# Lab-LVM/imagenet-models

Hardware: AMD Instinct MI355X
Metric: images/sec (whole node) GA-ConvNeXt-T 3x224x224 bf16 training step (higher is better)
Workload: dtype bf16; 1 GPU; ga_convnext_tiny_768 train step (fwd + GA loss lam=-0.8 + bwd + all-reduce + adamw lr=0), batch 256/GPU, drop_path 0.2, synthetic 3x224x224; global_batch=256, parallelism=dp1, dist_backend=none, grad_exchange=torch, allreduce_buckets=0

## Files before the change

imagenet-models_amd/_lib.py:

```python
import ctypes as C
import os

_HERE = os.path.dirname(os.path.abspath(__file__))
LIB_PATH = os.environ.get('GAEXT_LIB') or os.path.join(_HERE, 'csrc', 'libgaext.so')

GA_F32, GA_BF16 = 0, 1
ACT_NONE, ACT_GELU, ACT_RELU = 0, 1, 2
A_PLAIN, A_PATCH2, A_STEM4_NCHW, A_CONV3, A_CONV3S2, A_NEIGH2 = 0, 1, 2, 3, 4, 5
C_PLAIN, C_UNPATCH2 = 0, 1

vp, i32, i64, f32 = C.c_void_p, C.c_int, C.c_int64, C.c_float


class GemmDesc(C.Structure):
    _fields_ = [
        ('M', i32), ('N', i32), ('K', i32), ('batch', i32), ('dtype', i32),
        ('A', vp), ('lda', i64), ('strideA', i64), ('a_batch_mod', i32), ('a_kind', i32),
        ('a_H', i32), ('a_W', i32), ('a_C', i32), ('a_act', i32),
        ('B', vp), ('ldb', i64), ('strideB', i64),
        ('C', vp), ('ldc', i64), ('strideC', i64), ('c_kind', i32),
        ('c_H', i32), ('c_W', i32), ('c_C', i32), ('c_f32', i32), ('C2', vp), ('c2_mode', i32),
        ('alpha', f32), ('bias', vp), ('strideBias', i64), ('act', i32),
        ('H', vp), ('ldh', i64), ('strideH', i64), ('h_is_deriv', i32),
        ('rowscale', vp), ('rows_per_scale', i32),
# ... 123 lines not shown
    'ga_layernorm_bwd_dp': ([vp, vp, vp, vp, vp, vp, vp, vp, vp, i64, i32, i32, vp, vp, i64, i32, vp], i32),
    'ga_bn_finalize': ([vp, vp, i64, vp, vp, f32, f32, vp, vp, vp, vp, vp, vp, i32, i32, vp], i32),
    'ga_affine_act': ([vp, vp, vp, vp, vp, i64, vp, i64, i32, i32, i32, i64, vp], i32),
    'ga_bn_bwd_reduce': ([vp, vp, vp, vp, vp, vp, i64, vp, vp, i64, i32, i32, i64, vp], i32),
    'ga_bn_bwd_apply': ([vp, vp, vp, vp, vp, vp, vp, vp, vp, i64, i64, vp, i64, i32, i32, i64, i64, vp], i32),
    'ga_pool_concat_fwd': ([vp, vp, i32, i32, i32, i32, i32, i32, i32, i32, i32, i32, vp], i32),
    'ga_pool_concat_bwd': ([vp, vp, vp, i32, i32, i32, i32, i32, i32, i32, i32, i32, i32, vp], i32),
    'ga_spatial_sum': ([vp, vp, vp, i32, i32, i32, f32, i32, vp], i32),
    'ga_se_mlp_fwd': ([vp, vp, vp, vp, vp, vp, vp, i32, i32, i32, vp], i32),
    'ga_se_mlp_bwd': ([vp, vp, vp, vp, vp, vp, vp, f32, vp, vp, vp, vp, i32, i32, i32, vp], i32),
    'ga_chan_scale': ([vp, vp, vp, vp, i32, i32, i32, i32, vp], i32),
    'ga_gram_pack_fwd': ([vp, vp, vp, i32, i32, i32, i32, i32, vp], i32),
    'ga_gram_pack_bwd': ([vp, vp, vp, vp, i32, i32, i32, i32, i32, vp], i32),
    'ga_gram_f64_fwd_workspace': ([i32, i32], C.c_size_t),
    'ga_gram_f64_bwd_workspace': ([i32, i32], C.c_size_t),
    'ga_gram_f64_fwd': ([vp, vp, vp, vp, C.c_size_t, i32, i32, i32, i32, i32, i32, i32, vp], i32),
    'ga_gram_f64_bwd': ([vp, vp, vp, vp, vp, vp, C.c_size_t, i32, i32, i32, i32, i32, i32, i32, vp], i32),
    'ga_token_cat': ([vp, vp, vp, i32, i32, i32, i32, vp], i32),
    'ga_token_split': ([vp, vp, vp, i32, i32, i32, i32, i32, i32, vp], i32),
    'ga_class_attn_fwd': ([vp, vp, vp, vp, i32, i32, i32, i32, f32, i32, vp], i32),
    'ga_class_attn_bwd': ([vp, vp, vp, vp, vp, vp, i32, i32, i32, i32, f32, i32, vp], i32),
    'ga_class_attn_fwd2': ([vp, vp, vp, i64, vp, vp, i32, i32, i32, i32, f32, i32, vp], i32),
    'ga_class_attn_bwd2': ([vp, vp, vp, vp, i64, vp, vp, vp, vp, i32, i32, i32, i32, f32, i32, vp], i32),
    'ga_loss_fwd_bwd': ([vp, vp, vp, vp, i32, i32, i32, f32, i32, f32, f32, i32, vp], i32),
    'ga_heads_topk': ([vp, i32, i32, i32, i32, vp, vp, vp], i32),
    'ga_sgd_step': ([vp, vp, vp, vp, i64, i32, f32, vp], i32),
    'ga_adamw_step': ([vp, vp, vp, vp, vp, i64, f32, vp], i32),
    'ga_weight_prep_batch': ([vp, i32, vp], i32),
    'ga_weight_unfold_batch': ([vp, i32, vp], i32),
    'ga_small_batch': ([vp, i32, vp], i32),
    'ga_cswin_attn_fwd': ([C.POINTER(CswinAttnDesc), vp], i32),
    'ga_cswin_attn_bwd_workspace': ([C.POINTER(CswinAttnDesc)], C.c_size_t),
    'ga_cswin_attn_bwd': ([C.POINTER(CswinAttnDesc), vp, vp, vp, C.c_size_t, vp], i32),
    'ga_cswin_lepe_wgrad_reduce': ([C.POINTER(CswinAttnDesc), vp, vp, vp, vp, vp, vp], i32),
    'ga_cswin_lepe_wgrad': ([C.POINTER(CswinAttnDesc), vp, vp, vp, vp, vp, vp], i32),
    'ga_layernorm_gelu_fwd': ([vp, vp, vp, vp, vp, vp, i64, i32, f32, i32, vp], i32),
    'ga_layernorm_gelu_bwd': ([vp, vp, vp, vp, vp, vp, vp, vp, vp, i64, i32, i32, vp], i32),
    'ga_nchw3_to_nhwc8': ([vp, vp, i32, i32, i32, i32, vp], i32),
    'ga_convw_pack': ([vp, vp, i32, i32, i32, i32, i64, i32, vp], i32),
    'ga_convw_unpack_grad': ([vp, vp, i32, i32, i32, i32, i64, vp], i32),
    'ga_conv3s2_dgrad_prep': ([vp, vp, i32, i32, i64, i32, vp], i32),
    'ga_gram_pack_fwd2': ([vp, vp, vp, i32, i32, i32, i32, i32, i32, vp], i32),
    'ga_gram_pack_bwd2': ([vp, vp, vp, vp, i32, i32, i32, i32, i32, i32, vp], i32),
    'ga_map_tokens_fwd': ([vp, vp, i32, i32, i32, i32, i32, vp], i32),
    'ga_map_tokens_bwd': ([vp, vp, i32, i32, i32, i32, i32, vp], i32),
    'ga_class_attn_mt_fwd': ([vp, vp, vp, i64, vp, vp, vp, i32, i32, i32, i32, i32, f32, i32, vp], i32),
    'ga_class_attn_mt_bwd': ([vp, vp, vp, vp, i64, vp, vp, vp, vp, vp, i64, i32, i32, i32, i32, i32, f32, i32, vp], i32),
    'ga_class_attn_mt_ia_fwd': ([vp, vp, vp, i64, vp, vp, vp, vp, vp, vp, vp, i32, i32, i32, i32, i32, f32, i32, vp], i32),
    'ga_class_attn_mt_ia_bwd': ([vp, vp, vp, vp, i64, vp, vp, vp, vp, vp, vp, vp, vp, i64, vp, vp, vp, vp, i32, i32, i32, i32, i32, f32, i32,
                                 vp], i32),
    'ga_map_loss_fwd_bwd': ([vp, vp, vp, vp, vp, vp, i32, i32, i32, f32, i32, f32, f32, i32, vp], i32),
    'ga_gelu_fwd': ([vp, vp, i64, i32, vp], i32),
    'ga_gelu_bwd': ([vp, vp, vp, i64, i32, vp], i32),
    'ga_relu_drop': ([vp, vp, vp, vp, i64, i32, vp], i32),
    'ga_mask_mul': ([vp, vp, vp, vp, i64, i32, vp], i32),
    'ga_copy2d': ([vp, i64, vp, i64, i64, i32, i32, i32, vp], i32),
    'ga_dropout_mask_sample': ([vp, i64, f32, C.c_uint64, vp, vp], i32),
    'ga_drop_path_sample': ([vp, vp, i32, i32, C.c_uint64, vp, vp], i32),
    'ga_loss_dense_fwd_bwd': ([vp, vp, vp, vp, vp, vp, vp, i32, i32, i32, f32, i32, f32, f32, f32, i32, vp], i32),
    'ga_u8_normalize': ([vp, vp, i32, i32, i32, i32, C.POINTER(f32), C.POINTER(f32), vp], i32),
    'ga_input_erase': ([vp, i32, vp, i32, i32, i32, i32, C.POINTER(f32), C.POINTER(f32), vp, i32, i32, C.c_uint64, C.c_uint64, vp], i32),
    'ga_input_collate': ([vp, i32, vp, i32, i32, i32, i32, C.POINTER(f32), C.POINTER(f32), vp, vp, i32, i32, C.c_uint64, C.c_uint64, vp],
                         i32),
    'ga_mixup_target_elem': ([vp, vp, i32, i32, vp, C.c_double, vp], i32),
    'ga_rand_augment': ([vp, vp, vp, C.c_size_t, i32, i32, i32, i32, vp, i32, vp, vp], i32),
    'ga_rand_augment_work_bytes': ([i32, i32, i32, i32, i32], C.c_size_t),
    'ga_rand_augment_check_table': ([vp, i32], i32),
    'ga_resize_crop': ([vp, C.c_uint64, vp, vp, vp, C.c_size_t, i32, i32, i32, vp], i32),
    'ga_resize_crop_work_bytes': ([vp, i32, i32, i32], C.c_size_t),
    'ga_resize_crop_check_table': ([vp, i32, i32, i32, C.c_uint64], i32),
    'ga_resample_coeffs': ([i32, i32, i32, vp, vp, i32, vp], i32),
    'ga_jpeg_probe': ([vp, C.c_size_t, vp], i32),
    'ga_jpeg_entropy_decode': ([vp, C.c_size_t, vp, C.c_size_t, vp], i32),
    'ga_jpeg_check_table': ([vp, i32, C.c_uint64, C.c_uint64, C.c_uint64, C.c_uint64], i32),
    'ga_jpeg_work_bytes': ([vp, i32], C.c_size_t),
    'ga_jpeg_reconstruct': ([vp, i32, vp, vp, vp, vp, vp], i32),
    'ga_mixup_batch': ([vp, vp, i32, i32, i32, i32, C.c_double, i32, i32, i32, i32, i32, vp], i32),
    'ga_mixup_target': ([vp, vp, i32, i32, C.c_double, C.c_double, vp], i32),
    'ga_agc_clip': ([vp, vp, vp, i32, f32, f32, vp], i32),
    'ga_small_linear_fwd': ([C.POINTER(SmallLinearDesc), vp], i32),
    'ga_small_linear_bwd': ([C.POINTER(SmallLinearDesc), vp, vp, i32, vp, vp, vp, vp], i32),
    'ga_colstats': ([vp, i64, i32, i32, vp, vp, i32, vp], i32),
    'ga_pad_copy_f32': ([vp, vp, i64, i64, i64, i64, i32, vp], i32),
    'ga_pad_copy': ([vp, vp, i64, i64, i64, i64, i32, i32, vp], i32),
    'ga_stem4_ln_fwd': ([vp, vp, i64, vp, vp, vp, vp, vp, vp, vp, i32, i32, i32, i32, f32, vp], i32),
    'ga_blockdiag_f32': ([vp, vp, i64, i32, i32, i32, i64, i32, i32, vp], i32),
    'ga_pad_groups_f32': ([vp, vp, i64, i64, i32, i32, i32, i32, i32, i32, vp], i32),
    'ga_attn_fwd': ([C.POINTER(AttnDesc), vp], i32),
    'ga_attn_bwd_workspace': ([C.POINTER(AttnDesc)], C.c_size_t),
    'ga_attn_bwd': ([C.POINTER(AttnDesc), vp, vp, vp, C.c_size_t, vp], i32),
    'ga_patchify': ([vp, vp, i32, i32, i32, i32, i32, i32, vp], i32),
    'ga_vit_embed_fwd': ([vp, vp, vp, vp, i32, i32, i32, i32, vp], i32),
    'ga_vit_embed_bwd': ([vp, vp, vp, vp, i32, i32, i32, i32, vp], i32),
    'ga_patchify_strided': ([vp, vp, i32, i32, i32, i32, i32, i32, i32, vp], i32),
    'ga_pos_add_fwd': ([vp, vp, vp, i32, i32, i32, i32, vp], i32),
    'ga_pos_add_bwd': ([vp, vp, i32, i32, i32, i32, vp], i32),
    'ga_dwpool_fwd': ([vp, vp, vp, vp, i32, i32, i32, i32, i32, i32, vp], i32),
    'ga_dwpool_bwd_data': ([vp, vp, vp, i32, i32, i32, i32, i32, i32, vp], i32),
    'ga_dwpool_bwd_weight': ([vp, vp, vp, vp, i32, i32, i32, i32, i32, i32, vp], i32),
    'ga_resize_concat_fwd': ([vp, vp, i32, i32, i32, i32, i32, i32, i64, i32, i32, vp], i32),
    'ga_resize_concat_bwd': ([vp, vp, i32, i32, i32, i32, i32, i32, i64, i32, i32, vp], i32),
    'ga_rows_bcast': ([vp, vp, i32, i32, i32, f32, i32, vp], i32),
    'ga_token_gap_fwd': ([vp, vp, i32, i32, i32, i32, vp], i32),
    'ga_token_gap_bwd': ([vp, vp, i32, i32, i32, i32, vp], i32),
    'ga_mlp_supported': ([i32, i32, i32], i32),
    'ga_mlp_fwd': ([C.POINTER(MlpDesc), vp], i32),
    'ga_mlp_bwd': ([C.POINTER(MlpBwdDesc), vp], i32),
    'ga_mlp_bwd_wgrad_supported': ([i32, i32, i32], i32),
    'ga_mlp_bwd_partials': ([C.POINTER(MlpBwdDesc)], C.c_size_t),
    'ga_memset': ([vp, i32, C.c_size_t, vp], i32),
    'ga_transpose_f32': ([vp, vp, i32, i32, i32, vp], i32),
    'ga_axpy_f32': ([vp, vp, f32, i64, vp], i32),
    'ga_lerp_f32': ([vp, vp, f32, i64, vp], i32),
    'ga_sumsq_f32': ([vp, i64, vp, vp], i32),
    'ga_lamb_stage1': ([vp, vp, vp, vp, vp, vp, vp, vp, i32, vp, vp], i32),
    'ga_lamb_stage2': ([vp, vp, vp, vp, i32, vp, vp], i32),
    'ga_clip_grad_f32': ([vp, i64, vp, f32, i32, vp], i32),
    'ga_rowscale': ([vp, vp, vp, i64, i64, i32, vp], i32),
    'ga_cast_from_f32': ([vp, vp, i64, i32, vp], i32),
    'ga_cast_to_f32': ([vp, vp, i64, i32, vp], i32),
}

_lib = None


def load():
    global _lib
    if _lib is not None:
        return _lib
    if not os.path.exists(LIB_PATH):
        raise RuntimeError(f'libgaext.so not found at {LIB_PATH}: build it with `make -C {os.path.dirname(LIB_PATH)}` '
                           f'(there is no CPU fallback for the product path)')
    lib = C.CDLL(LIB_PATH)
    for name, (argtypes, restype) in _SIGS.items():
        fn = getattr(lib, name)
        fn.argtypes = argtypes
        fn.restype = restype
    _lib = lib
    return lib


def last_error():
    buf = C.create_string_buffer(512)
    load().ga_last_error(buf, 512)
    return buf.value.decode(errors='replace')


def config_string():
    buf = C.create_string_buffer(1024)
    load().ga_config_string(buf, 1024)
    s = buf.value.decode(errors='replace')
    host = sorted(k for k in os.environ if k.startswith(('GAEXT_', 'GA_FUSED_MLP')) and k != 'GAEXT_LIB')
    known = {'GAEXT_ASYNC_WGRAD', 'GAEXT_FWD_SPLIT', 'GAEXT_PAR_BRANCH', 'GAEXT_FWD_SKEW', 'GAEXT_FUSE_DP', 'GAEXT_HEAD_STREAMS',
             'GA_FUSED_MLP', 'GAEXT_SMALL_SINGLE', 'GAEXT_SYNC_DEBUG', 'GAEXT_MLP_WG1', 'GAEXT_MLP_PREFETCH'}
    for k in host:
        if k in known:
            s += f' host:{k}={os.environ[k]}'
    if os.environ.get('GAEXT_LIB'):
        s += f' lib={os.environ["GAEXT_LIB"]}'
    return s


class knobs:

    def __init__(self, **kv):
        self.kv = kv

    def __enter__(self):
        lib = load()
        for k, v in self.kv.items():
            check(lib.ga_set_knob(k.encode(), int(v)), f'ga_set_knob({k})')
        return self

    def __exit__(self, *exc):
        lib = load()
        for k in self.kv:
            lib.ga_unset_knob(k.encode())
        return False


def check(rc, what):
    if rc != 0:
        raise RuntimeError(f'libgaext {what} failed (code {rc}): {last_error()}')


def exported_symbols():
    return sorted(_SIGS)
```

imagenet-models_amd/csrc/wprep.hip:

```cpp
#include <algorithm>
#include "common.h"

namespace {

__device__ __forceinline__ long w_index(int n, int kcol, int Ci, int KH, int KW, int stem, int* ci_out) {
    const int KK = Ci * KH * KW;
    if (stem || (KH == 1 && KW == 1)) {
        *ci_out = stem ? kcol / (KH * KW) : kcol;
        return (long)n * KK + kcol;
    }
    const int tap = kcol / Ci, ci = kcol - tap * Ci;
    *ci_out = ci;
    return ((long)n * Ci + ci) * (KH * KW) + tap;
}

template <typename T>
__global__ __launch_bounds__(256) void wprep_out_kernel(const float* __restrict__ w, const float* __restrict__ rs,
                                                        const float* __restrict__ cs, const int* __restrict__ perm,
                                                        T* __restrict__ out, long ldo, int rows, int Ci, int KH, int KW,
                                                        int stem) {
    const int KK = Ci * KH * KW;
    const long total = (long)rows * ldo;
    for (long i = (long)blockIdx.x * 256 + threadIdx.x; i < total; i += (long)gridDim.x * 256) {
        const int no = (int)(i / ldo), kcol = (int)(i - (long)no * ldo);
// ... 301 lines not shown
            const long t = i / tcols;
            const int r = (int)(t % trows), g = (int)(t / trows);
            float v = 0.f;
            if (!d.flip) {
                if (col < d.Co) {
                    const int n = d.row_perm ? d.row_perm[g * d.Co + col] : g * d.Co + col;
                    int ci;
                    v = d.w[w_index(n, r, d.Ci, d.KH, d.KW, d.stem, &ci)];
                    if (d.rs) v *= d.rs[n];
                    if (d.cs) v *= d.cs[ci];
                }
            } else if (col < d.KH * d.KW * d.Co) {
                const int tapf = col / d.Co, co = col - tapf * d.Co;
                const int tap = d.KH * d.KW - 1 - tapf;
                const int n = d.row_perm ? d.row_perm[g * d.Co + co] : g * d.Co + co;
                v = d.w[((long)n * d.Ci + r) * (d.KH * d.KW) + tap];
                if (d.rs) v *= d.rs[n];
                if (d.cs) v *= d.cs[r];
            }
            elt<T>::st(outT + t * d.ldt + col, v);
        }
    }
}

__global__ __launch_bounds__(256) void wprep_batch_kernel(const ga_wprep_desc* __restrict__ jobs) {
    __shared__ float tile[64][65];
    const ga_wprep_desc d = jobs[blockIdx.y];
    if (wprep_is_1x1(d)) {
        if (d.dtype == GA_BF16) wprep_job_1x1<bf16_t>(d, gridDim.x, blockIdx.x, tile);
        else wprep_job_1x1<float>(d, gridDim.x, blockIdx.x, tile);
        return;
    }
    if (d.dtype == GA_BF16) wprep_job<bf16_t>(d, gridDim.x, blockIdx.x);
    else wprep_job<float>(d, gridDim.x, blockIdx.x);
}

__global__ __launch_bounds__(256) void small_batch_kernel(const ga_small_desc* __restrict__ jobs) {
    const ga_small_desc d = jobs[blockIdx.y];
    if (d.kind == 0) {
        for (long i = (long)blockIdx.x * 256 + threadIdx.x; i < d.n; i += (long)gridDim.x * 256) d.y[i] += d.a * d.x[i];
    } else if (d.kind == 1) {
        const long total = (long)d.R * d.C;
        for (long i = (long)blockIdx.x * 256 + threadIdx.x; i < total; i += (long)gridDim.x * 256) {
            const int c = (int)(i / d.R), r = (int)(i - (long)c * d.R);
            const float v = d.x[(long)r * d.C + c];
            d.y[i] = d.accumulate ? d.y[i] + v : v;
        }
    } else {
        const int lane = threadIdx.x & 63;
        for (int no = blockIdx.x * 4 + (threadIdx.x >> 6); no < d.R; no += gridDim.x * 4) {
            const int n = d.row_perm ? d.row_perm[no] : no;
            float s = 0.f;
            if (d.v) {
                if (d.C % 4 == 0 && ((reinterpret_cast<uintptr_t>(d.x) | reinterpret_cast<uintptr_t>(d.v)) & 15) == 0) {
                    for (int c = lane * 4; c < d.C; c += 256) {
                        float w[4], vv[4];
                        load4(d.x + (long)n * d.C + c, w);
                        load4(d.v + c, vv);
                        s += w[0] * vv[0] + w[1] * vv[1] + w[2] * vv[2] + w[3] * vv[3];
                    }
                } else {
                    for (int c = lane; c < d.C; c += 64) s += d.x[(long)n * d.C + c] * d.v[c];
                }
            }
            s = wave_sum(s);
            if (lane == 0) d.y[no] = (d.rs ? d.rs[n] : 1.f) * ((d.b ? d.b[n] : 0.f) + s);
        }
    }
}

__global__ __launch_bounds__(256) void unfold_batch_kernel(const ga_wunfold_desc* __restrict__ jobs) {
    const ga_wunfold_desc d = jobs[blockIdx.y];
    const int KK = d.Ci * d.KH * d.KW;
    const bool vec4 = d.KH == 1 && d.KW == 1 && !d.stem && KK % 4 == 0 && d.ldg % 4 == 0 &&
                      ((reinterpret_cast<uintptr_t>(d.G) | reinterpret_cast<uintptr_t>(d.dW) |
                        reinterpret_cast<uintptr_t>(d.cs) | reinterpret_cast<uintptr_t>(d.v)) & 15) == 0;
    if (d.dW && vec4) {
        const unsigned P = (unsigned)KK >> 2, total = (unsigned)d.N * P;
        for (unsigned i = blockIdx.x * 256u + threadIdx.x; i < total; i += gridDim.x * 256u) {
            const unsigned no = i / P, k4 = (i - no * P) << 2;
            const int n = d.row_perm ? d.row_perm[no] : (int)no;
            float g[4], w[4];
            load4(d.G + (long)no * d.ldg + k4, g);
            if (d.cs) {
                float cs[4];
                load4(d.cs + k4, cs);
#pragma unroll
                for (int j = 0; j < 4; ++j) g[j] *= cs[j];
            }
            if (d.gb && d.v) {
                float vv[4];
                load4(d.v + k4, vv);
                const float gbn = d.gb[no];
#pragma unroll
                for (int j = 0; j < 4; ++j) g[j] = fmaf(gbn, vv[j], g[j]);
            }
            const float rs = d.rs ? d.rs[n] : 1.f;
            float* dst = d.dW + (long)n * KK + k4;
            load4(dst, w);
#pragma unroll
            for (int j = 0; j < 4; ++j) w[j] = fmaf(g[j], rs, w[j]);
            store4(dst, w);
        }
    } else if (d.dW) {
        const long total = (long)d.N * KK;
        for (long i = (long)blockIdx.x * 256 + threadIdx.x; i < total; i += (long)gridDim.x * 256) {
            const int no = (int)(i / KK), kcol = (int)(i - (long)no * KK);
            const int n = d.row_perm ? d.row_perm[no] : no;
            int ci;
            const long wi = w_index(n, kcol, d.Ci, d.KH, d.KW, d.stem, &ci);
            float val = d.G[(long)no * d.ldg + kcol];
            if (d.cs) val *= d.cs[ci];
            if (d.gb && d.v) val += d.gb[no] * d.v[ci];
            if (d.rs) val *= d.rs[n];
            d.dW[wi] += val;
        }
    }
    if (d.d_rs || (d.db && d.gb)) {
        const int lane = threadIdx.x & 63;
        for (int no = blockIdx.x * 4 + (threadIdx.x >> 6); no < d.N; no += gridDim.x * 4) {
            const int n = d.row_perm ? d.row_perm[no] : no;
            if (d.d_rs) {
                float s = 0.f;
                for (int k = lane; k < KK; k += 64) {
                    int ci;
                    const long wi = w_index(n, k, d.Ci, d.KH, d.KW, d.stem, &ci);
                    s += d.G[(long)no * d.ldg + k] * d.W[wi] * (d.cs ? d.cs[ci] : 1.f);
                    if (d.gb && d.v) s += d.gb[no] * d.W[wi] * d.v[ci];
                }
                s = wave_sum(s);
                if (lane == 0) d.d_rs[n] += s + ((d.gb && d.b) ? d.gb[no] * d.b[n] : 0.f);
            }
            if (d.db && d.gb && lane == 0) d.db[n] += (d.rs ? d.rs[n] : 1.f) * d.gb[no];
        }
    }
    if (d.d_cs || d.d_v) {
        const int rows_per_blk = (d.N + gridDim.x - 1) / gridDim.x;
        const int r0 = blockIdx.x * rows_per_blk, r1 = min(d.N, r0 + rows_per_blk);
        for (int c = threadIdx.x; c < d.Ci; c += 256) {
            float a = 0.f, bs = 0.f;
            for (int n = r0; n < r1; ++n) {
                const float wv = d.W[(long)n * d.Ci + c] * (d.rs ? d.rs[n] : 1.f);
                a += d.G[(long)n * d.ldg + c] * wv;
                if (d.gb) bs += d.gb[n] * wv;
            }
            if (r1 > r0) {
                if (d.d_cs) atomicAdd(d.d_cs + c, a);
                if (d.d_v) atomicAdd(d.d_v + c, bs);
            }
        }
    }
}

int nblocks(long n, int cap = 4096) { return (int)std::max<long>(1, std::min<long>(cap, (n + 255) / 256)); }

}

extern "C" int ga_weight_prep(const ga_wprep_desc* d, ga_stream_t stream) {
    GA_REQUIRE(d && d->w && d->G >= 1 && d->Co >= 1 && d->Ci >= 1 && d->KH >= 1 && d->KW >= 1, "ga_weight_prep: bad args");
    GA_REQUIRE(!(d->cs && d->G > 1), "ga_weight_prep: column scale with groups unsupported");
    GA_REQUIRE(!(d->flip && d->stem), "ga_weight_prep: flip+stem unsupported");
    GA_REQUIRE(d->t_cols == 0 || d->t_cols == d->ldt, "ga_weight_prep: t_cols != ldt needs ga_weight_prep_batch");
    const int KK = d->Ci * d->KH * d->KW;
    hipStream_t s = reinterpret_cast<hipStream_t>(stream);
    if (d->out) {
        GA_REQUIRE(d->ldo >= KK, "ga_weight_prep: ldo < K");
        const long total = (long)d->G * d->Co * d->ldo;
        if (d->dtype == GA_BF16)
            hipLaunchKernelGGL(wprep_out_kernel<bf16_t>, dim3(nblocks(total)), dim3(256), 0, s, d->w, d->rs, d->cs,
                               d->row_perm, (bf16_t*)d->out, (long)d->ldo, d->G * d->Co, d->Ci, d->KH, d->KW, d->stem);
        else
            hipLaunchKernelGGL(wprep_out_kernel<float>, dim3(nblocks(total)), dim3(256), 0, s, d->w, d->rs, d->cs,
                               d->row_perm, (float*)d->out, (long)d->ldo, d->G * d->Co, d->Ci, d->KH, d->KW, d->stem);
    }
    if (d->outT) {
        GA_REQUIRE(d->ldt >= (d->flip ? d->KH * d->KW * d->Co : d->Co), "ga_weight_prep: ldt too small");
        const long total = (long)d->G * (d->flip ? d->Ci : KK) * d->ldt;
        if (d->dtype == GA_BF16)
            hipLaunchKernelGGL(wprep_outT_kernel<bf16_t>, dim3(nblocks(total)), dim3(256), 0, s, d->w, d->rs, d->cs,
                               d->row_perm, (bf16_t*)d->outT, (long)d->ldt, d->G, d->Co, d->Ci, d->KH, d->KW, d->stem, d->flip);
        else
            hipLaunchKernelGGL(wprep_outT_kernel<float>, dim3(nblocks(total)), dim3(256), 0, s, d->w, d->rs, d->cs,
                               d->row_perm, (float*)d->outT, (long)d->ldt, d->G, d->Co, d->Ci, d->KH, d->KW, d->stem, d->flip);
    }
    return ga_check_launch("ga_weight_prep");
}

extern "C" int ga_bias_fold(const float* W, const float* b, const float* rs, const float* v, const int* row_perm,
                            float* be, int N, int C, ga_stream_t stream) {
    GA_REQUIRE(be && N > 0 && (!v || W), "ga_bias_fold: bad args");
    hipLaunchKernelGGL(bias_fold_kernel, dim3(cdiv(N, 4)), dim3(256), 0, reinterpret_cast<hipStream_t>(stream), W, b, rs,
                       v, row_perm, be, N, C);
    return ga_check_launch("ga_bias_fold");
}

extern "C" int ga_weight_unfold(const ga_wunfold_desc* d, ga_stream_t stream) {
    GA_REQUIRE(d && d->G && d->N > 0 && d->Ci > 0, "ga_weight_unfold: bad args");
    GA_REQUIRE(!((d->d_cs || d->d_v || d->v) && (d->KH != 1 || d->KW != 1)),
               "ga_weight_unfold: column grads / bias-fold vector need a 1x1 kernel");
    GA_REQUIRE(!((d->d_rs || d->d_cs || d->d_v) && !d->W), "ga_weight_unfold: W required");
    GA_REQUIRE(!(d->row_perm && (d->d_cs || d->d_v)), "ga_weight_unfold: row_perm with column grads unsupported");
    hipStream_t s = reinterpret_cast<hipStream_t>(stream);
    const int KK = d->Ci * d->KH * d->KW;
    if (d->dW)
        hipLaunchKernelGGL(unfold_dw_kernel, dim3(nblocks((long)d->N * KK)), dim3(256), 0, s, d->G, (long)d->ldg, d->rs,
                           d->cs, d->gb, d->v, d->row_perm, d->dW, d->N, d->Ci, d->KH, d->KW, d->stem);
    if (d->d_rs || (d->db && d->gb))
        hipLaunchKernelGGL(unfold_rows_kernel, dim3(cdiv(d->N, 4)), dim3(256), 0, s, d->G, (long)d->ldg, d->gb, d->W,
                           d->b, d->rs, d->cs, d->v, d->row_perm, d->d_rs, d->db, d->N, d->Ci, d->KH, d->KW, d->stem);
    if (d->d_cs || d->d_v)
        hipLaunchKernelGGL(unfold_cols_kernel, dim3(cdiv(d->Ci, 64), cdiv(d->N, 64)), dim3(256), 0, s, d->G,
                           (long)d->ldg, d->gb, d->W, d->rs, d->d_cs, d->d_v, d->N, d->Ci);
    return ga_check_launch("ga_weight_unfold");
}

extern "C" int ga_transpose_f32(const float* in, float* out, int R, int C, int accumulate, ga_stream_t stream) {
    GA_REQUIRE(in && out && R > 0 && C > 0, "ga_transpose_f32: bad args");
    hipLaunchKernelGGL(transpose_f32_kernel, dim3(nblocks((long)R * C)), dim3(256), 0,
                       reinterpret_cast<hipStream_t>(stream), in, out, R, C, accumulate);
    return ga_check_launch("ga_transpose_f32");
}

extern "C" int ga_axpy_f32(float* y, const float* x, float a, int64_t n, ga_stream_t stream) {
    GA_REQUIRE(y && x && n > 0, "ga_axpy_f32: bad args");
    hipLaunchKernelGGL(axpy_f32_kernel, dim3(nblocks(n)), dim3(256), 0, reinterpret_cast<hipStream_t>(stream), y, x, a,
                       (long)n);
    return ga_check_launch("ga_axpy_f32");
}

extern "C" int ga_lerp_f32(float* y, const float* x, float w, int64_t n, ga_stream_t stream) {
    GA_REQUIRE(y && x && n > 0, "ga_lerp_f32: bad args");
    hipLaunchKernelGGL(lerp_f32_kernel, dim3(nblocks(n)), dim3(256), 0, reinterpret_cast<hipStream_t>(stream), y, x, w,
                       (long)n);
    return ga_check_launch("ga_lerp_f32");
}

extern "C" int ga_rowscale(const void* x, const float* s, void* y, int64_t n, int64_t elems_per_scale, int dtype,
                           ga_stream_t stream) {
    GA_REQUIRE(x && s && y && n > 0 && n % 8 == 0 && elems_per_scale % 8 == 0, "ga_rowscale: bad args");
    hipStream_t st = reinterpret_cast<hipStream_t>(stream);
    if (dtype == GA_BF16)
        hipLaunchKernelGGL(rowscale_kernel<bf16_t>, dim3(nblocks(n / 8 / 4, 2048)), dim3(256), 0, st, (const bf16_t*)x, s,
                           (bf16_t*)y, (long)(n / 8), (long)elems_per_scale);
    else
        hipLaunchKernelGGL(rowscale_kernel<float>, dim3(nblocks(n / 8 / 2, 2048)), dim3(256), 0, st, (const float*)x, s,
                           (float*)y, (long)(n / 8), (long)elems_per_scale);
    return ga_check_launch("ga_rowscale");
}

extern "C" int ga_cast_from_f32(const float* src, void* dst, int64_t n, int dtype, ga_stream_t stream) {
    GA_REQUIRE(src && dst && n > 0, "ga_cast_from_f32: bad args");
    hipStream_t st = reinterpret_cast<hipStream_t>(stream);
    if (dtype == GA_BF16)
        hipLaunchKernelGGL(cast_kernel<bf16_t>, dim3(nblocks(n)), dim3(256), 0, st, src, (bf16_t*)dst, (long)n);
    else
        hipLaunchKernelGGL(cast_kernel<float>, dim3(nblocks(n)), dim3(256), 0, st, src, (float*)dst, (long)n);
    return ga_check_launch("ga_cast_from_f32");
}

extern "C" int ga_cast_to_f32(const void* src, float* dst, int64_t n, int dtype, ga_stream_t stream) {
    GA_REQUIRE(src && dst && n > 0, "ga_cast_to_f32: bad args");
    hipStream_t st = reinterpret_cast<hipStream_t>(stream);
    if (dtype == GA_BF16)
        hipLaunchKernelGGL(uncast_kernel<bf16_t>, dim3(nblocks(n)), dim3(256), 0, st, (const bf16_t*)src, dst, (long)n);
    else
        hipLaunchKernelGGL(uncast_kernel<float>, dim3(nblocks(n)), dim3(256), 0, st, (const float*)src, dst, (long)n);
    return ga_check_launch("ga_cast_to_f32");
}

extern "C" int ga_weight_prep_batch(const ga_wprep_desc* jobs_dev, int n, ga_stream_t stream) {
    GA_REQUIRE(jobs_dev && n > 0, "ga_weight_prep_batch: bad args");
    const int gx = std::max(1, GA_KNOB("BATCH_GX", 256));
    hipLaunchKernelGGL(wprep_batch_kernel, dim3(gx, n), dim3(256), 0, reinterpret_cast<hipStream_t>(stream), jobs_dev);
    return ga_check_launch("ga_weight_prep_batch");
}

extern "C" int ga_small_batch(const ga_small_desc* jobs_dev, int n, ga_stream_t stream) {
    GA_REQUIRE(jobs_dev && n > 0, "ga_small_batch: bad args");
    hipLaunchKernelGGL(small_batch_kernel, dim3(48, n), dim3(256), 0, reinterpret_cast<hipStream_t>(stream), jobs_dev);
    return ga_check_launch("ga_small_batch");
}

extern "C" int ga_weight_unfold_batch(const ga_wunfold_desc* jobs_dev, int n, ga_stream_t stream) {
    GA_REQUIRE(jobs_dev && n > 0, "ga_weight_unfold_batch: bad args");
    const int gx = std::max(1, GA_KNOB("BATCH_GX", 256));
    hipLaunchKernelGGL(unfold_batch_kernel, dim3(gx, n), dim3(256), 0, reinterpret_cast<hipStream_t>(stream), jobs_dev);
    return ga_check_launch("ga_weight_unfold_batch");
}
```

Measured before the change: 11150 images/sec.

## Add load-balanced persistent v2 kernels for batched small and weight-unfold jobs

Adds v2 kernels for the batched small-op and weight-unfold gradient jobs. A persistent grid sized to the CU count walks a prefix-summed tile list across all jobs, replacing the fixed grid of one block row per job. The unfold path adds specialised tile modes: vectorised 1x1 tiles with LDS column reductions, and an LDS-transposed mode for multi-tap convolution weights. Some reductions now accumulate in double precision. The new path is on by default through the WPREP_V2 knob, and it adds binary-search scheduling overhead and more code-path complexity.

```diff
diff --git a/imagenet-models_amd/_lib.py b/imagenet-models_amd/_lib.py
--- a/imagenet-models_amd/_lib.py
+++ b/imagenet-models_amd/_lib.py
@@ -299,7 +299,8 @@
     s = buf.value.decode(errors='replace')
     host = sorted(k for k in os.environ if k.startswith(('GAEXT_', 'GA_FUSED_MLP')) and k != 'GAEXT_LIB')
     known = {'GAEXT_ASYNC_WGRAD', 'GAEXT_FWD_SPLIT', 'GAEXT_PAR_BRANCH', 'GAEXT_FWD_SKEW', 'GAEXT_FUSE_DP', 'GAEXT_HEAD_STREAMS',
-             'GA_FUSED_MLP', 'GAEXT_SMALL_SINGLE', 'GAEXT_SYNC_DEBUG', 'GAEXT_MLP_WG1', 'GAEXT_MLP_PREFETCH'}
+             'GA_FUSED_MLP', 'GAEXT_SMALL_SINGLE', 'GAEXT_SYNC_DEBUG', 'GAEXT_MLP_WG1', 'GAEXT_MLP_PREFETCH',
+             'GAEXT_WPREP_V2'}
     for k in host:
         if k in known:
             s += f' host:{k}={os.environ[k]}'
diff --git a/imagenet-models_amd/csrc/wprep.hip b/imagenet-models_amd/csrc/wprep.hip
--- a/imagenet-models_amd/csrc/wprep.hip
+++ b/imagenet-models_amd/csrc/wprep.hip
@@ -477,6 +477,465 @@
     }
 }
 
+constexpr int V2_JOBS = 256;
+constexpr int V2_FLAT = 4096;
+constexpr int V2_SPAN = 144;
+constexpr int V2_LDW = V2_SPAN + 1;
+
+struct v2_sched {
+    unsigned pref[V2_JOBS + 1];
+    unsigned wsum[4];
+};
+
+template <typename Desc, typename Count, typename Run>
+__device__ __forceinline__ void v2_walk(const Desc* __restrict__ jobs, int n, v2_sched& sc, Count count, Run run) {
+    const int lane = threadIdx.x & 63, wave = threadIdx.x >> 6;
+    unsigned base = 0;
+    for (int j0 = 0; j0 < n; j0 += V2_JOBS) {
+        const int nj = min(V2_JOBS, n - j0);
+        unsigned v = (int)threadIdx.x < nj ? count(jobs[j0 + threadIdx.x]) : 0u;
+#pragma unroll
+        for (int o = 1; o < 64; o <<= 1) {
+            const unsigned u = __shfl_up(v, o, 64);
+            if (lane >= o) v += u;
+        }
+        __syncthreads();
+        if (lane == 63) sc.wsum[wave] = v;
+        __syncthreads();
+        for (int w = 0; w < wave; ++w) v += sc.wsum[w];
+        sc.pref[threadIdx.x + 1] = v;
+        if (threadIdx.x == 0) sc.pref[0] = 0;
+        __syncthreads();
+        const unsigned total = sc.pref[V2_JOBS];
+        for (unsigned t = (blockIdx.x + gridDim.x - base % gridDim.x) % gridDim.x; t < total; t += gridDim.x) {
+            int lo = 0, hi = nj;
+            while (hi - lo > 1) {
+                const int mid = (lo + hi) >> 1;
+                if (sc.pref[mid] <= t) lo = mid;
+                else hi = mid;
+            }
+            lo = __builtin_amdgcn_readfirstlane(lo);
+            run(j0 + lo, (int)(t - sc.pref[lo]));
+        }
+        base += total;
+    }
+}
+
+__device__ __forceinline__ bool al16(const void* p) { return (reinterpret_cast<uintptr_t>(p) & 15) == 0; }
+
+__device__ __forceinline__ float dot4_unfused(const float w[4], const float v[4]) {
+#pragma clang fp contract(off)
+    const float p0 = w[0] * v[0], p1 = w[1] * v[1], p2 = w[2] * v[2], p3 = w[3] * v[3];
+    return ((p0 + p1) + p2) + p3;
+}
+__device__ __forceinline__ unsigned small_v2_tiles(const ga_small_desc& d) {
+    if (d.kind == 0) return (unsigned)((d.n + V2_FLAT - 1) / V2_FLAT);
+    if (d.kind == 1) return (unsigned)(((d.R + 31) >> 5) * ((d.C + 31) >> 5));
+    return (unsigned)((d.R + 3) >> 2);
+}
+
+__global__ __launch_bounds__(256) void small_batch_v2_kernel(const ga_small_desc* __restrict__ jobs, int n) {
+    __shared__ float tile[32][33];
+    __shared__ v2_sched sc;
+    v2_walk(jobs, n, sc, [](const ga_small_desc& d) { return small_v2_tiles(d); }, [&](int j, int t) {
+        const ga_small_desc d = jobs[j];
+        if (d.kind == 0) {
+            const long i0 = (long)t * V2_FLAT, end = std::min((long)d.n, i0 + V2_FLAT);
+            if (al16(d.x) && al16(d.y)) {
+                float x[4][4], y[4][4];
+#pragma unroll
+                for (int u = 0; u < 4; ++u) {
+                    const long i = i0 + (u * 256 + (int)threadIdx.x) * 4;
+                    if (i + 4 <= end) load4(d.x + i, x[u]), load4(d.y + i, y[u]);
+                }
+#pragma unroll
+                for (int u = 0; u < 4; ++u) {
+                    const long i = i0 + (u * 256 + (int)threadIdx.x) * 4;
+                    if (i + 4 <= end) {
+#pragma unroll
+                        for (int e = 0; e < 4; ++e) y[u][e] += d.a * x[u][e];
+                        store4(d.y + i, y[u]);
+                    } else {
+                        for (long k = i; k < end; ++k) d.y[k] += d.a * d.x[k];
+                    }
+                }
+            } else {
+                for (long i = i0 + threadIdx.x; i < end; i += 256) d.y[i] += d.a * d.x[i];
+            }
+        } else if (d.kind == 1) {
+            const int tc = (d.C + 31) >> 5;
+            const int r0 = (t / tc) << 5, c0 = (t % tc) << 5;
+            const int rw = min(32, d.R - r0), cw = min(32, d.C - c0), ne = rw * cw;
+            float v[4], y[4];
+#pragma unroll
+            for (int u = 0; u < 4; ++u) {
+                const int idx = threadIdx.x + 256 * u, ri = idx / cw, ci = idx - ri * cw;
+                const int yc = idx / rw, yr = idx - yc * rw;
+                v[u] = idx < ne ? d.x[(long)(r0 + ri) * d.C + c0 + ci] : 0.f;
+                y[u] = (idx < ne && d.accumulate) ? d.y[(long)(c0 + yc) * d.R + r0 + yr] : 0.f;
+            }
+#pragma unroll
+            for (int u = 0; u < 4; ++u) {
+                const int idx = threadIdx.x + 256 * u, ri = idx / cw, ci = idx - ri * cw;
+                if (idx < ne) tile[ri][ci] = v[u];
+            }
+            __syncthreads();
+#pragma unroll
+            for (int u = 0; u < 4; ++u) {
+                const int idx = threadIdx.x + 256 * u, ci = idx / rw, ri = idx - ci * rw;
+                if (idx < ne) d.y[(long)(c0 + ci) * d.R + r0 + ri] = d.accumulate ? y[u] + tile[ri][ci] : tile[ri][ci];
+            }
+            __syncthreads();
+        } else {
+            const int lane = threadIdx.x & 63;
+            const int no = t * 4 + (threadIdx.x >> 6);
+            if (no < d.R) {
+                const int m = d.row_perm ? d.row_perm[no] : no;
+                float s = 0.f;
+                if (d.v) {
+                    if (d.C % 4 == 0 && ((reinterpret_cast<uintptr_t>(d.x) | reinterpret_cast<uintptr_t>(d.v)) & 15) == 0) {
+                        for (int c = lane * 4; c < d.C; c += 1024) {
+                            float w[4][4], vv[4][4];
+#pragma unroll
+                            for (int u = 0; u < 4; ++u)
+                                if (c + 256 * u < d.C) load4(d.x + (long)m * d.C + c + 256 * u, w[u]), load4(d.v + c + 256 * u, vv[u]);
+#pragma unroll
+                            for (int u = 0; u < 4; ++u)
+                                if (c + 256 * u < d.C) s += dot4_unfused(w[u], vv[u]);
+                        }
+                    } else {
+                        for (int c = lane; c < d.C; c += 64) s += d.x[(long)m * d.C + c] * d.v[c];
+                    }
+                }
+                s = wave_sum(s);
+                if (lane == 0) d.y[no] = (d.rs ? d.rs[m] : 1.f) * ((d.b ? d.b[m] : 0.f) + s);
+            }
+        }
+    });
+}
+
+struct unfold_v2_plan {
+    int mode, K, tk, cb;
+    unsigned t1, t2, t3;
+};
+
+__device__ __forceinline__ unfold_v2_plan unfold_v2_plan_of(const ga_wunfold_desc& d) {
+    unfold_v2_plan p = {};
+    const int KK2 = d.KH * d.KW, KK = d.Ci * KK2;
+    const bool dbs = d.db && d.gb, rows = d.d_rs || dbs, cols = d.d_cs || d.d_v;
+    const bool al = d.ldg % 4 == 0 && al16(d.G) && al16(d.dW) && al16(d.cs) && al16(d.v);
+    const unsigned r4 = (unsigned)((d.N + 3) >> 2);
+    p.K = KK;
+    if (al && KK % 4 == 0 && KK2 == 1 && !d.stem && (!(d.d_rs || cols) || al16(d.W))) {
+        p.mode = 1, p.tk = (KK + 63) >> 6;
+        const unsigned t64 = (unsigned)(((d.N + 63) >> 6) * p.tk);
+        if (d.d_rs) p.t2 = r4, p.t3 = cols ? t64 : 0u;
+        else p.t1 = (d.dW || cols || dbs) ? t64 : 0u;
+        return p;
+    }
+    if (al && !d.stem && KK2 > 1 && d.Ci % 4 == 0 && d.dW && !d.cs && !d.v && !cols) {
+        p.cb = min(16, (V2_SPAN / KK2) & ~3);
+        if (p.cb >= 4) {
+            p.mode = 2, p.tk = (d.Ci + p.cb - 1) / p.cb;
+            p.t1 = (unsigned)(((d.N + 63) >> 6) * p.tk);
+            p.t2 = rows ? r4 : 0u;
+            return p;
+        }
+    }
+    p.t1 = d.dW ? (unsigned)(((long)d.N * KK + V2_FLAT - 1) / V2_FLAT) : 0u;
+    p.t2 = rows ? r4 : 0u;
+    p.t3 = cols ? (unsigned)((d.N + 63) >> 6) : 0u;
+    return p;
+}
+
+__device__ __forceinline__ void unfold_v2_tile_1x1(const ga_wunfold_desc& d, const unfold_v2_plan& p, int t, bool elem, bool cols,
+                                                   float* lds) {
+    double(*red)[16][64] = reinterpret_cast<double(*)[16][64]>(lds);
+    const int K = p.K;
+    const int tr = threadIdx.x >> 4, tc = threadIdx.x & 15;
+    const int r0 = (t / p.tk) << 6, kcol = ((t % p.tk) << 6) + tc * 4;
+    const bool dwp = elem && d.dW;
+    double a[4] = {0., 0., 0., 0.}, bs[4] = {0., 0., 0., 0.};
+    if (kcol < K) {
+        float g[4][4], w[4][4], dw[4][4], rs[4], gbn[4];
+        int nn[4];
+#pragma unroll
+        for (int i = 0; i < 4; ++i) {
+            const int no = r0 + tr + 16 * i;
+            if (no >= d.N) continue;
+            const int n = nn[i] = d.row_perm ? d.row_perm[no] : no;
+            load4(d.G + (long)no * d.ldg + kcol, g[i]);
+            if (cols) load4(d.W + (long)n * K + kcol, w[i]);
+            if (dwp) load4(d.dW + (long)n * K + kcol, dw[i]);
+            rs[i] = d.rs ? d.rs[n] : 1.f;
+            gbn[i] = d.gb ? d.gb[no] : 0.f;
+        }
+        float cs[4] = {1.f, 1.f, 1.f, 1.f}, vv[4] = {0.f, 0.f, 0.f, 0.f};
+        if (dwp && d.cs) load4(d.cs + kcol, cs);
+        if (dwp && d.gb && d.v) load4(d.v + kcol, vv);
+#pragma unroll
+        for (int i = 0; i < 4; ++i) {
+            if (r0 + tr + 16 * i >= d.N) continue;
+            if (cols) {
+#pragma unroll
+                for (int j = 0; j < 4; ++j) {
+                    const double wv = (double)w[i][j] * rs[i];
+                    a[j] += g[i][j] * wv;
+                    if (d.gb) bs[j] += gbn[i] * wv;
+                }
+            }
+            if (dwp) {
+#pragma unroll
+                for (int j = 0; j < 4; ++j) {
+                    float e = g[i][j];
+                    if (d.cs) e *= cs[j];
+                    if (d.gb && d.v) e = fmaf(gbn[i], vv[j], e);
+                    dw[i][j] = fmaf(e, rs[i], dw[i][j]);
+                }
+                store4(d.dW + (long)nn[i] * K + kcol, dw[i]);
+            }
+        }
+    }
+    if (elem && d.db && d.gb && !d.d_rs && tc == 0 && t % p.tk == 0) {
+#pragma unroll
+        for (int i = 0; i < 4; ++i) {
+            const int no = r0 + tr + 16 * i;
+            if (no < d.N) {
+                const int n = d.row_perm ? d.row_perm[no] : no;
+                d.db[n] += (d.rs ? d.rs[n] : 1.f) * d.gb[no];
+            }
+        }
+    }
+    if (cols) {
+#pragma unroll
+        for (int j = 0; j < 4; ++j) red[0][tr][tc * 4 + j] = a[j], red[1][tr][tc * 4 + j] = bs[j];
+        __syncthreads();
+        if (threadIdx.x < 128) {
+            const int which = threadIdx.x >> 6, c = threadIdx.x & 63;
+            double s = 0.;
+#pragma unroll
+            for (int i = 0; i < 16; ++i) s += red[which][i][c];
+            float* dst = which ? d.d_v : d.d_cs;
+            const int col = ((t % p.tk) << 6) + c;
+            if (dst && col < K) atomicAdd(dst + col, (float)s);
+        }
+        __syncthreads();
+    }
+}
+
+__device__ __forceinline__ void unfold_v2_tile_rows(const ga_wunfold_desc& d, const unfold_v2_plan& p, int t) {
+    const int K = p.K, lane = threadIdx.x & 63;
+    const int no = t * 4 + (threadIdx.x >> 6);
+    if (no >= d.N) return;
+    const bool bias = d.gb && d.v;
+    const int n = d.row_perm ? d.row_perm[no] : no;
+    const float rs = d.rs ? d.rs[n] : 1.f, gbn = d.gb ? d.gb[no] : 0.f;
+    double s = 0.;
+    for (int k0 = lane * 4; k0 < K; k0 += 1024) {
+        float g[4][4], w[4][4], dw[4][4];
+#pragma unroll
+        for (int u = 0; u < 4; ++u) {
+            const int k = k0 + 256 * u;
+            if (k >= K) continue;
+            load4(d.G + (long)no * d.ldg + k, g[u]);
+            if (d.d_rs) load4(d.W + (long)n * K + k, w[u]);
+            if (d.dW) load4(d.dW + (long)n * K + k, dw[u]);
+        }
+#pragma unroll
+        for (int u = 0; u < 4; ++u) {
+            const int k = k0 + 256 * u;
+            if (k >= K) continue;
+            float cs[4] = {1.f, 1.f, 1.f, 1.f}, vv[4] = {0.f, 0.f, 0.f, 0.f};
+            if (d.cs) load4(d.cs + k, cs);
+            if (bias) load4(d.v + k, vv);
+            if (d.d_rs) {
+#pragma unroll
+                for (int j = 0; j < 4; ++j) {
+                    s += (double)g[u][j] * w[u][j] * cs[j];
+                    if (bias) s += (double)gbn * w[u][j] * vv[j];
+                }
+            }
+            if (d.dW) {
+#pragma unroll
+                for (int j = 0; j < 4; ++j) {
+                    float e = g[u][j];
+                    if (d.cs) e *= cs[j];
+                    if (bias) e = fmaf(gbn, vv[j], e);
+                    dw[u][j] = fmaf(e, rs, dw[u][j]);
+                }
+                store4(d.dW + (long)n * K + k, dw[u]);
+            }
+        }
+    }
+    if (d.d_rs) {
+#pragma unroll
+        for (int o = 32; o > 0; o >>= 1) s += __shfl_xor(s, o, 64);
+        if (lane == 0) d.d_rs[n] += (float)s + ((d.gb && d.b) ? gbn * d.b[n] : 0.f);
+    }
+    if (d.db && d.gb && lane == 0) d.db[n] += rs * gbn;
+}
+
+__device__ __forceinline__ void unfold_v2_tile_taps(const ga_wunfold_desc& d, const unfold_v2_plan& p, int t, float* lds) {
+    const int KK2 = d.KH * d.KW, Ci = d.Ci;
+    const int r0 = (t / p.tk) << 6, c0 = (t % p.tk) * p.cb;
+    const int cb = min(p.cb, Ci - c0), cb4 = cb >> 2;
+    const int rows = min(64, d.N - r0), S4 = (cb * KK2) >> 2;
+    const int n1 = rows * KK2 * cb4, n2 = rows * S4;
+    for (int b = threadIdx.x; b < n1; b += 1024) {
+        float g[4][4];
+#pragma unroll
+        for (int u = 0; u < 4; ++u) {
+            const int idx = b + 256 * u;
+            if (idx >= n1) continue;
+            const int cq = idx % cb4, rt = idx / cb4;
+            const int tap = rt % KK2, row = rt / KK2;
+            load4(d.G + (long)(r0 + row) * d.ldg + tap * Ci + c0 + cq * 4, g[u]);
+        }
+#pragma unroll
+        for (int u = 0; u < 4; ++u) {
+            const int idx = b + 256 * u;
+            if (idx >= n1) continue;
+            const int cq = idx % cb4, rt = idx / cb4;
+            const int tap = rt % KK2, row = rt / KK2;
+#pragma unroll
+            for (int j = 0; j < 4; ++j) lds[row * V2_LDW + (cq * 4 + j) * KK2 + tap] = g[u][j];
+        }
+    }
+    __syncthreads();
+    for (int b = threadIdx.x; b < n2; b += 1024) {
+        float w[4][4], rs[4];
+#pragma unroll
+        for (int u = 0; u < 4; ++u) {
+            const int idx = b + 256 * u;
+            if (idx >= n2) continue;
+            const int row = idx / S4, q = idx - row * S4;
+            const int n = d.row_perm ? d.row_perm[r0 + row] : r0 + row;
+            load4(d.dW + ((long)n * Ci + c0) * KK2 + q * 4, w[u]);
+            rs[u] = d.rs ? d.rs[n] : 1.f;
+        }
+#pragma unroll
+        for (int u = 0; u < 4; ++u) {
+            const int idx = b + 256 * u;
+            if (idx >= n2) continue;
+            const int row = idx / S4, q = idx - row * S4;
+            const int n = d.row_perm ? d.row_perm[r0 + row] : r0 + row;
+#pragma unroll
+            for (int j = 0; j < 4; ++j) {
+                float val = lds[row * V2_LDW + q * 4 + j];
+                if (d.rs) val *= rs[u];
+                w[u][j] += val;
+            }
+            store4(d.dW + ((long)n * Ci + c0) * KK2 + q * 4, w[u]);
+        }
+    }
+    __syncthreads();
+}
+
+__device__ __forceinline__ void unfold_v2_flat_dw(const ga_wunfold_desc& d, int KK, int t) {
+    const bool vec4 = d.KH == 1 && d.KW == 1 && !d.stem && KK % 4 == 0 && d.ldg % 4 == 0 && al16(d.G) && al16(d.dW) &&
+                      al16(d.cs) && al16(d.v);
+    if (vec4) {
+        const unsigned P = (unsigned)KK >> 2, total = (unsigned)d.N * P, end = min(total, ((unsigned)t + 1) * (V2_FLAT / 4));
+        for (unsigned i = (unsigned)t * (V2_FLAT / 4) + threadIdx.x; i < end; i += 256) {
+            const unsigned no = i / P, k4 = (i - no * P) << 2;
+            const int n = d.row_perm ? d.row_perm[no] : (int)no;
+            float g[4], w[4];
+            load4(d.G + (long)no * d.ldg + k4, g);
+            if (d.cs) {
+                float cs[4];
+                load4(d.cs + k4, cs);
+#pragma unroll
+                for (int j = 0; j < 4; ++j) g[j] *= cs[j];
+            }
+            if (d.gb && d.v) {
+                float vv[4];
+                load4(d.v + k4, vv);
+                const float gbn = d.gb[no];
+#pragma unroll
+                for (int j = 0; j < 4; ++j) g[j] = fmaf(gbn, vv[j], g[j]);
+            }
+            const float rs = d.rs ? d.rs[n] : 1.f;
+            float* dst = d.dW + (long)n * KK + k4;
+            load4(dst, w);
+#pragma unroll
+            for (int j = 0; j < 4; ++j) w[j] = fmaf(g[j], rs, w[j]);
+            store4(dst, w);
+        }
+        return;
+    }
+    const long total = (long)d.N * KK, end = std::min(total, ((long)t + 1) * V2_FLAT);
+    for (long i = (long)t * V2_FLAT + threadIdx.x; i < end; i += 256) {
+        const int no = (int)(i / KK), kcol = (int)(i - (long)no * KK);
+        const int n = d.row_perm ? d.row_perm[no] : no;
+        int ci;
+        const long wi = w_index(n, kcol, d.Ci, d.KH, d.KW, d.stem, &ci);
+        float val = d.G[(long)no * d.ldg + kcol];
+        if (d.cs) val *= d.cs[ci];
+        if (d.gb && d.v) val += d.gb[no] * d.v[ci];
+        if (d.rs) val *= d.rs[n];
+        d.dW[wi] += val;
+    }
+}
+__device__ __forceinline__ void unfold_v2_flat_rows(const ga_wunfold_desc& d, int KK, int t) {
+    const int lane = threadIdx.x & 63;
+    const int no = t * 4 + (threadIdx.x >> 6);
+    if (no >= d.N) return;
+    const int n = d.row_perm ? d.row_perm[no] : no;
+    if (d.d_rs) {
+        float s = 0.f;
+        for (int k = lane; k < KK; k += 64) {
+            int ci;
+            const long wi = w_index(n, k, d.Ci, d.KH, d.KW, d.stem, &ci);
+            s += d.G[(long)no * d.ldg + k] * d.W[wi] * (d.cs ? d.cs[ci] : 1.f);
+            if (d.gb && d.v) s += d.gb[no] * d.W[wi] * d.v[ci];
+        }
+        s = wave_sum(s);
+        if (lane == 0) d.d_rs[n] += s + ((d.gb && d.b) ? d.gb[no] * d.b[n] : 0.f);
+    }
+    if (d.db && d.gb && lane == 0) d.db[n] += (d.rs ? d.rs[n] : 1.f) * d.gb[no];
+}
+__device__ __forceinline__ void unfold_v2_flat_cols(const ga_wunfold_desc& d, int t) {
+    const int r0 = t * 64, r1 = min(d.N, r0 + 64);
+    for (int c = threadIdx.x; c < d.Ci; c += 256) {
+        double a = 0., bs = 0.;
+        for (int n = r0; n < r1; ++n) {
+            const double wv = (double)d.W[(long)n * d.Ci + c] * (d.rs ? d.rs[n] : 1.f);
+            a += d.G[(long)n * d.ldg + c] * wv;
+            if (d.gb) bs += d.gb[n] * wv;
+        }
+        if (d.d_cs) atomicAdd(d.d_cs + c, (float)a);
+        if (d.d_v) atomicAdd(d.d_v + c, (float)bs);
+    }
+}
+
+__global__ __launch_bounds__(256) void unfold_batch_v2_kernel(const ga_wunfold_desc* __restrict__ jobs, int n) {
+    __shared__ __align__(16) float lds[64 * V2_LDW];
+    __shared__ v2_sched sc;
+    v2_walk(jobs, n, sc,
+            [](const ga_wunfold_desc& d) {
+                const unfold_v2_plan p = unfold_v2_plan_of(d);
+                return p.t1 + p.t2 + p.t3;
+            },
+            [&](int j, int t) {
+                const ga_wunfold_desc d = jobs[j];
+                const unfold_v2_plan p = unfold_v2_plan_of(d);
+                const unsigned u = (unsigned)t;
+                if (u < p.t1) {
+                    if (p.mode == 1) unfold_v2_tile_1x1(d, p, t, true, d.d_cs || d.d_v, lds);
+                    else if (p.mode == 2) unfold_v2_tile_taps(d, p, t, lds);
+                    else unfold_v2_flat_dw(d, p.K, t);
+                } else if (u < p.t1 + p.t2) {
+                    if (p.mode == 1) unfold_v2_tile_rows(d, p, t - (int)p.t1);
+                    else unfold_v2_flat_rows(d, p.K, t - (int)p.t1);
+                } else {
+                    if (p.mode == 1) unfold_v2_tile_1x1(d, p, t - (int)(p.t1 + p.t2), false, true, lds);
+                    else unfold_v2_flat_cols(d, t - (int)(p.t1 + p.t2));
+                }
+            });
+}
+
+int v2_grid(int per_cu) { return ga_num_cus() * per_cu; }
+
 int nblocks(long n, int cap = 4096) { return (int)std::max<long>(1, std::min<long>(cap, (n + 255) / 256)); }
 
 }
@@ -602,12 +1061,20 @@
 
 extern "C" int ga_small_batch(const ga_small_desc* jobs_dev, int n, ga_stream_t stream) {
     GA_REQUIRE(jobs_dev && n > 0, "ga_small_batch: bad args");
+    if (GA_KNOB("WPREP_V2", 1)) {
+        hipLaunchKernelGGL(small_batch_v2_kernel, dim3(v2_grid(4)), dim3(256), 0, reinterpret_cast<hipStream_t>(stream), jobs_dev, n);
+        return ga_check_launch("ga_small_batch");
+    }
     hipLaunchKernelGGL(small_batch_kernel, dim3(48, n), dim3(256), 0, reinterpret_cast<hipStream_t>(stream), jobs_dev);
     return ga_check_launch("ga_small_batch");
 }
 
 extern "C" int ga_weight_unfold_batch(const ga_wunfold_desc* jobs_dev, int n, ga_stream_t stream) {
     GA_REQUIRE(jobs_dev && n > 0, "ga_weight_unfold_batch: bad args");
+    if (GA_KNOB("WPREP_V2", 1)) {
+        hipLaunchKernelGGL(unfold_batch_v2_kernel, dim3(v2_grid(3)), dim3(256), 0, reinterpret_cast<hipStream_t>(stream), jobs_dev, n);
+        return ga_check_launch("ga_weight_unfold_batch");
+    }
     const int gx = std::max(1, GA_KNOB("BATCH_GX", 256));
     hipLaunchKernelGGL(unfold_batch_kernel, dim3(gx, n), dim3(256), 0, reinterpret_cast<hipStream_t>(stream), jobs_dev);
     return ga_check_launch("ga_weight_unfold_batch");
```

Measured after the change: 11120 images/sec. Within noise of the previous version (-0.3%).
